# mit-acl/clipper

Hardware: AMD Instinct MI355X
Metric: affinity+solve ms and GEMV HBM GB/s, n=10k assoc, 95% outliers, 1/8 GPU (lower is better)
Workload: dtype f64 (M stored f32)

## Files before the change

### clipper_amd/csrc/k_affinity.hip.h

```cpp
#pragma once

#include <hip/hip_runtime.h>
#include <stdint.h>

#include "k_csc.hip.h"

namespace clipper_hip {


__global__ __launch_bounds__(256) void k_gather_points(const double* __restrict__ D, int d,
                                                        const int32_t* __restrict__ idx,
                                                        int64_t m, int64_t pstride,
                                                        double* __restrict__ P,
                                                        float* __restrict__ Pf) {
  const int64_t i = static_cast<int64_t>(blockIdx.x) * 256 + threadIdx.x;
  if (i >= pstride) return;
  const int64_t src = (i < m) ? idx[i] : 0;
  for (int k = 0; k < d; ++k) {
    const double v = (i < m) ? D[k + d * src] : 0.0;
    P[k * pstride + i] = v;
    Pf[k * pstride + i] = static_cast<float>(v);
  }
}

template <typename T>
__device__ __forceinline__ T store_score(double scr, double affinityeps) {
  if (!(scr > affinityeps)) return T(0);
  T v = static_cast<T>(scr);
  if (v == T(0)) v = static_cast<T>(1.17549435e-38);
  return v;
}

template <typename T>
__device__ __forceinline__ void store4(T* p, T a, T b, T c, T d);
template <>
__device__ __forceinline__ void store4<float>(float* p, float a, float b, float c, float d) {
  *reinterpret_cast<float4*>(p) = make_float4(a, b, c, d);
}
template <>
__device__ __forceinline__ void store4<double>(double* p, double a, double b, double c,
                                               double d) {
  *reinterpret_cast<double4*>(p) = make_double4(a, b, c, d);
}

struct EuclidParams {
  double sigma, epsilon, mindist, affinityeps;
};

template <typename T, int D>
__global__ __launch_bounds__(256) void k_affinity_euclid(
    T* __restrict__ S, int64_t ld, int64_t m, int64_t c0, int rows_per_blk, int d,
    const double* __restrict__ P1, const double* __restrict__ P2, int64_t pstride,
    const int32_t* __restrict__ A0, const int32_t* __restrict__ A1, EuclidParams prm) {
  const int64_t c = (static_cast<int64_t>(blockIdx.x) * 256 + threadIdx.x) * 4;
  if (c >= ld) return;
  const int64_t r0 = static_cast<int64_t>(blockIdx.y) * rows_per_blk;
  const int64_t r1 = (r0 + rows_per_blk < m) ? r0 + rows_per_blk : m;
  constexpr int DD = (D > 0) ? D : 1;

  int64_t gi[4];
  bool valid[4];
  int32_t a0c[4], a1c[4];
  double p1c[4][DD], p2c[4][DD];
#pragma unroll
  for (int q = 0; q < 4; ++q) {
    const int64_t g = c0 + c + q;
    valid[q] = g < m;
    gi[q] = valid[q] ? g : (m - 1);
    a0c[q] = A0[gi[q]];
    a1c[q] = A1[gi[q]];
    if (D > 0) {
#pragma unroll
      for (int k = 0; k < DD; ++k) {
        p1c[q][k] = P1[k * pstride + gi[q]];
        p2c[q][k] = P2[k * pstride + gi[q]];
      }
    }
  }

  for (int64_t r = r0; r < r1; ++r) {
    const int32_t a0r = A0[r], a1r = A1[r];
    double p1r[DD], p2r[DD];
    if (D > 0) {
#pragma unroll
      for (int k = 0; k < DD; ++k) {
        p1r[k] = P1[k * pstride + r];
        p2r[k] = P2[k * pstride + r];
      }
    }
    T out[4];
#pragma unroll
    for (int q = 0; q < 4; ++q) {
      double s1 = 0.0, s2 = 0.0;
      if (D > 0) {
#pragma unroll
        for (int k = 0; k < DD; ++k) {
          const double t1 = p1r[k] - p1c[q][k];
          const double t2 = p2r[k] - p2c[q][k];
          s1 = fma(t1, t1, s1);
          s2 = fma(t2, t2, s2);
        }
      } else {
        for (int k = 0; k < d; ++k) {
          const double t1 = P1[k * pstride + r] - P1[k * pstride + gi[q]];
          const double t2 = P2[k * pstride + r] - P2[k * pstride + gi[q]];
          s1 = fma(t1, t1, s1);
          s2 = fma(t2, t2, s2);
        }
      }
      const double l1 = sqrt(s1), l2 = sqrt(s2);
      bool ok = valid[q] && (a0r != a0c[q]) && (a1r != a1c[q]);
      if (prm.mindist > 0 && (l1 < prm.mindist || l2 < prm.mindist)) ok = false;
      const double cc = fabs(l1 - l2);
      double scr = 0.0;
      if (ok && cc < prm.epsilon) scr = exp(-0.5 * cc * cc / (prm.sigma * prm.sigma));
      out[q] = store_score<T>(scr, prm.affinityeps);
    }
    store4<T>(S + r * ld + c, out[0], out[1], out[2], out[3]);
  }
}

struct PointNormalParams {
  double sigp, epsp, sign, epsn, affinityeps;
};

template <typename T>
__global__ __launch_bounds__(256) void k_affinity_pointnormal(
    T* __restrict__ S, int64_t ld, int64_t m, int64_t c0, int rows_per_blk,
    const double* __restrict__ P1, const double* __restrict__ P2, int64_t pstride,
    const int32_t* __restrict__ A0, const int32_t* __restrict__ A1, PointNormalParams prm) {
  const int64_t c = (static_cast<int64_t>(blockIdx.x) * 256 + threadIdx.x) * 4;
  if (c >= ld) return;
  const int64_t r0 = static_cast<int64_t>(blockIdx.y) * rows_per_blk;
  const int64_t r1 = (r0 + rows_per_blk < m) ? r0 + rows_per_blk : m;

  bool valid[4];
  int32_t a0c[4], a1c[4];
  double p1c[4][6], p2c[4][6];
#pragma unroll
  for (int q = 0; q < 4; ++q) {
    const int64_t g = c0 + c + q;
    valid[q] = g < m;
    const int64_t gi = valid[q] ? g : (m - 1);
    a0c[q] = A0[gi];
    a1c[q] = A1[gi];
#pragma unroll
    for (int k = 0; k < 6; ++k) {
      p1c[q][k] = P1[k * pstride + gi];
      p2c[q][k] = P2[k * pstride + gi];
    }
  }

  for (int64_t r = r0; r < r1; ++r) {
    const int32_t a0r = A0[r], a1r = A1[r];
    double p1r[6], p2r[6];
#pragma unroll
    for (int k = 0; k < 6; ++k) {
      p1r[k] = P1[k * pstride + r];
      p2r[k] = P2[k * pstride + r];
    }
    T out[4];
#pragma unroll
    for (int q = 0; q < 4; ++q) {
      double s1 = 0.0, s2 = 0.0;
#pragma unroll
      for (int k = 0; k < 3; ++k) {
        const double t1 = p1r[k] - p1c[q][k];
        const double t2 = p2r[k] - p2c[q][k];
        s1 = fma(t1, t1, s1);
        s2 = fma(t2, t2, s2);
      }
      const double l1 = sqrt(s1), l2 = sqrt(s2);
      const double dot1 = fma(p1r[5], p1c[q][5], fma(p1r[4], p1c[q][4], p1r[3] * p1c[q][3]));
      const double dot2 = fma(p2r[5], p2c[q][5], fma(p2r[4], p2c[q][4], p2r[3] * p2c[q][3]));
      const bool ok = valid[q] && (a0r != a0c[q]) && (a1r != a1c[q]);
      double scr = 0.0;
      if (ok) {
        const double alpha1 = acos(dot1);
        const double alpha2 = acos(dot2);
        const double dp = fabs(l1 - l2);
        const double dn = fabs(alpha1 - alpha2);
        if (dp < prm.epsp && dn < prm.epsn) {
          const double sp = exp(-0.5 * dp * dp / (prm.sigp * prm.sigp));
          const double sn = exp(-0.5 * dn * dn / (prm.sign * prm.sign));
          scr = sp * sn;
        }
      }
      out[q] = store_score<T>(scr, prm.affinityeps);
    }
    store4<T>(S + r * ld + c, out[0], out[1], out[2], out[3]);
  }
}


constexpr int AFF_RG = 8;

__device__ __forceinline__ uint32_t lane_prefix(uint64_t mask) {
  return __builtin_amdgcn_mbcnt_hi(static_cast<uint32_t>(mask >> 32),
                                   __builtin_amdgcn_mbcnt_lo(static_cast<uint32_t>(mask), 0u));
}

__device__ __forceinline__ double pt_at(const double* __restrict__ P, uint32_t byte_off) {
  return *reinterpret_cast<const double*>(reinterpret_cast<const char*>(P) + byte_off);
}

template <typename T, int D>
__device__ __forceinline__ double exact_euclid_score(const double* __restrict__ P1,
                                                     const double* __restrict__ P2,
                                                     int64_t pstride, int64_t r, int64_t g,
                                                     const EuclidParams& prm) {
  const uint32_t pb = static_cast<uint32_t>(pstride) << 3, rb = static_cast<uint32_t>(r) << 3, gb = static_cast<uint32_t>(g) << 3;
  double s1 = 0.0, s2 = 0.0;
#pragma unroll
  for (int k = 0; k < D; ++k) {
    const double t1 = pt_at(P1, k * pb + rb) - pt_at(P1, k * pb + gb);
    const double t2 = pt_at(P2, k * pb + rb) - pt_at(P2, k * pb + gb);
    s1 = fma(t1, t1, s1);
    s2 = fma(t2, t2, s2);
  }
  const double l1 = sqrt(s1), l2 = sqrt(s2);
  if (prm.mindist > 0 && (l1 < prm.mindist || l2 < prm.mindist)) return 0.0;
  const double cc = fabs(l1 - l2);
  return (cc < prm.epsilon) ? exp(-0.5 * cc * cc / (prm.sigma * prm.sigma)) : 0.0;
}

template <typename T, int D>
__global__ __launch_bounds__(256) void k_affinity_euclid_compact(
    T* __restrict__ S, int64_t ld, int64_t m, int64_t c0, int rows_per_blk,
    const double* __restrict__ P1, const double* __restrict__ P2,
    const float* __restrict__ P1f, const float* __restrict__ P2f, int64_t pstride,
    const int32_t* __restrict__ A0, const int32_t* __restrict__ A1, EuclidParams prm,
    float eps_guarded) {
  __shared__ uint32_t queue[4][AFF_RG * 256];
  __shared__ T stage[4][AFF_RG][256];
  const int lane = threadIdx.x & 63;
  const int wave = __builtin_amdgcn_readfirstlane(threadIdx.x >> 6);
  const int64_t cw = static_cast<int64_t>(blockIdx.x) * 1024 + wave * 256;
  const int64_t c = cw + lane * 4;
  const int64_t r0 = static_cast<int64_t>(blockIdx.y) * rows_per_blk;
  const int64_t r1 = (r0 + rows_per_blk < m) ? r0 + rows_per_blk : m;
  if (cw >= ld) return;

  bool valid[4];
  int32_t a0c[4], a1c[4];
  float p1c[4][D], p2c[4][D];
#pragma unroll
  for (int q = 0; q < 4; ++q) {
    const int64_t g = c0 + c + q;
    valid[q] = (g < m) && (c + q < ld);
    const int64_t gi = (g < m) ? g : (m - 1);
    a0c[q] = A0[gi];
    a1c[q] = A1[gi];
#pragma unroll
    for (int k = 0; k < D; ++k) {
      p1c[q][k] = P1f[k * pstride + gi];
      p2c[q][k] = P2f[k * pstride + gi];
    }
  }
#pragma unroll
  for (int r8 = 0; r8 < AFF_RG; ++r8)
#pragma unroll
    for (int q = 0; q < 4; ++q) stage[wave][r8][lane * 4 + q] = T(0);

  for (int64_t base = r0; base < r1; base += AFF_RG) {
    uint32_t count = 0;
#pragma unroll
    for (int r8 = 0; r8 < AFF_RG; ++r8) {
      const int64_t r = base + r8;
      if (r < r1) {
        const int32_t a0r = A0[r], a1r = A1[r];
        float p1r[D], p2r[D];
#pragma unroll
        for (int k = 0; k < D; ++k) {
          p1r[k] = P1f[k * pstride + r];
          p2r[k] = P2f[k * pstride + r];
        }
#pragma unroll
        for (int q = 0; q < 4; ++q) {
          float s1 = 0.f, s2 = 0.f;
#pragma unroll
          for (int k = 0; k < D; ++k) {
            const float t1 = p1r[k] - p1c[q][k];
            const float t2 = p2r[k] - p2c[q][k];
            s1 = fmaf(t1, t1, s1);
            s2 = fmaf(t2, t2, s2);
          }
          const float cf = fabsf(__builtin_amdgcn_sqrtf(s1) - __builtin_amdgcn_sqrtf(s2));
          const bool cand = valid[q] && (a0r != a0c[q]) && (a1r != a1c[q]) && (cf < eps_guarded);
          const uint64_t mask = __ballot(cand);
          if (mask != 0) {
            if (cand) queue[wave][count + lane_prefix(mask)] =
                (static_cast<uint32_t>(r8) << 16) | static_cast<uint32_t>(lane * 4 + q);
            count += static_cast<uint32_t>(__popcll(mask));
          }
        }
      }
    }
    __builtin_amdgcn_fence(__ATOMIC_RELEASE, "wavefront");
    __builtin_amdgcn_wave_barrier();
    for (uint32_t e = lane; e < count; e += 64) {
      const uint32_t code = queue[wave][e];
      const int r8 = static_cast<int>(code >> 16);
      const int cl = static_cast<int>(code & 0xffffu);
      const double scr = exact_euclid_score<T, D>(P1, P2, pstride, base + r8, c0 + cw + cl, prm);
      stage[wave][r8][cl] = store_score<T>(scr, prm.affinityeps);
    }
    __builtin_amdgcn_fence(__ATOMIC_RELEASE, "wavefront");
    __builtin_amdgcn_wave_barrier();
    if (c < ld) {
#pragma unroll
      for (int r8 = 0; r8 < AFF_RG; ++r8) {
        const int64_t r = base + r8;
        if (r < r1) {
          T* sp = &stage[wave][r8][lane * 4];
          store4<T>(S + r * ld + c, sp[0], sp[1], sp[2], sp[3]);
          sp[0] = sp[1] = sp[2] = sp[3] = T(0);
        }
      }
    }
    __builtin_amdgcn_fence(__ATOMIC_RELEASE, "wavefront");
    __builtin_amdgcn_wave_barrier();
  }
}

template <typename T>
__device__ __forceinline__ double exact_pointnormal_score(const double* __restrict__ P1,
                                                          const double* __restrict__ P2,
                                                          int64_t pstride, int64_t r, int64_t g,
                                                          const PointNormalParams& prm) {
  const uint32_t pb = static_cast<uint32_t>(pstride) << 3, rb = static_cast<uint32_t>(r) << 3, gb = static_cast<uint32_t>(g) << 3;
  double p1r[6], p1g[6], p2r[6], p2g[6];
#pragma unroll
  for (int k = 0; k < 6; ++k) {
    p1r[k] = pt_at(P1, k * pb + rb);
    p1g[k] = pt_at(P1, k * pb + gb);
    p2r[k] = pt_at(P2, k * pb + rb);
    p2g[k] = pt_at(P2, k * pb + gb);
  }
  double s1 = 0.0, s2 = 0.0;
#pragma unroll
  for (int k = 0; k < 3; ++k) {
    const double t1 = p1r[k] - p1g[k];
    const double t2 = p2r[k] - p2g[k];
    s1 = fma(t1, t1, s1);
    s2 = fma(t2, t2, s2);
  }
  const double l1 = sqrt(s1), l2 = sqrt(s2);
  const double dot1 = fma(p1r[5], p1g[5], fma(p1r[4], p1g[4], p1r[3] * p1g[3]));
  const double dot2 = fma(p2r[5], p2g[5], fma(p2r[4], p2g[4], p2r[3] * p2g[3]));
  const double alpha1 = acos(dot1);
  const double alpha2 = acos(dot2);
  const double dp = fabs(l1 - l2);
  const double dn = fabs(alpha1 - alpha2);
  if (dp < prm.epsp && dn < prm.epsn) {
    const double sp = exp(-0.5 * dp * dp / (prm.sigp * prm.sigp));
    const double sn = exp(-0.5 * dn * dn / (prm.sign * prm.sign));
    return sp * sn;
  }
  return 0.0;
}

template <typename T>
__global__ __launch_bounds__(256) void k_affinity_pointnormal_compact(
    T* __restrict__ S, int64_t ld, int64_t m, int64_t c0, int rows_per_blk,
    const double* __restrict__ P1, const double* __restrict__ P2,
    const float* __restrict__ P1f, const float* __restrict__ P2f, int64_t pstride,
    const int32_t* __restrict__ A0, const int32_t* __restrict__ A1, PointNormalParams prm,
    float eps_guarded) {
  __shared__ uint32_t queue[4][AFF_RG * 256];
  __shared__ T stage[4][AFF_RG][256];
  const int lane = threadIdx.x & 63;
  const int wave = __builtin_amdgcn_readfirstlane(threadIdx.x >> 6);
  const int64_t cw = static_cast<int64_t>(blockIdx.x) * 1024 + wave * 256;
  const int64_t c = cw + lane * 4;
  const int64_t r0 = static_cast<int64_t>(blockIdx.y) * rows_per_blk;
  const int64_t r1 = (r0 + rows_per_blk < m) ? r0 + rows_per_blk : m;
  if (cw >= ld) return;

  bool valid[4];
  int32_t a0c[4], a1c[4];
  float p1c[4][3], p2c[4][3];
#pragma unroll
  for (int q = 0; q < 4; ++q) {
    const int64_t g = c0 + c + q;
    valid[q] = (g < m) && (c + q < ld);
    const int64_t gi = (g < m) ? g : (m - 1);
    a0c[q] = A0[gi];
    a1c[q] = A1[gi];
#pragma unroll
    for (int k = 0; k < 3; ++k) {
      p1c[q][k] = P1f[k * pstride + gi];
      p2c[q][k] = P2f[k * pstride + gi];
    }
  }
#pragma unroll
  for (int r8 = 0; r8 < AFF_RG; ++r8)
#pragma unroll
    for (int q = 0; q < 4; ++q) stage[wave][r8][lane * 4 + q] = T(0);

  for (int64_t base = r0; base < r1; base += AFF_RG) {
    uint32_t count = 0;
#pragma unroll
    for (int r8 = 0; r8 < AFF_RG; ++r8) {
      const int64_t r = base + r8;
      if (r < r1) {
        const int32_t a0r = A0[r], a1r = A1[r];
        float p1r[3], p2r[3];
#pragma unroll
        for (int k = 0; k < 3; ++k) {
          p1r[k] = P1f[k * pstride + r];
          p2r[k] = P2f[k * pstride + r];
        }
#pragma unroll
        for (int q = 0; q < 4; ++q) {
          float s1 = 0.f, s2 = 0.f;
#pragma unroll
          for (int k = 0; k < 3; ++k) {
            const float t1 = p1r[k] - p1c[q][k];
            const float t2 = p2r[k] - p2c[q][k];
            s1 = fmaf(t1, t1, s1);
            s2 = fmaf(t2, t2, s2);
          }
          const float dpf = fabsf(__builtin_amdgcn_sqrtf(s1) - __builtin_amdgcn_sqrtf(s2));
          const bool cand = valid[q] && (a0r != a0c[q]) && (a1r != a1c[q]) && (dpf < eps_guarded);
          const uint64_t mask = __ballot(cand);
          if (mask != 0) {
            if (cand) queue[wave][count + lane_prefix(mask)] =
                (static_cast<uint32_t>(r8) << 16) | static_cast<uint32_t>(lane * 4 + q);
            count += static_cast<uint32_t>(__popcll(mask));
          }
        }
      }
    }
    __builtin_amdgcn_fence(__ATOMIC_RELEASE, "wavefront");
    __builtin_amdgcn_wave_barrier();
    for (uint32_t e = lane; e < count; e += 64) {
      const uint32_t code = queue[wave][e];
      const int r8 = static_cast<int>(code >> 16);
      const int cl = static_cast<int>(code & 0xffffu);
      const double scr = exact_pointnormal_score<T>(P1, P2, pstride, base + r8, c0 + cw + cl, prm);
      stage[wave][r8][cl] = store_score<T>(scr, prm.affinityeps);
    }
    __builtin_amdgcn_fence(__ATOMIC_RELEASE, "wavefront");
    __builtin_amdgcn_wave_barrier();
    if (c < ld) {
#pragma unroll
      for (int r8 = 0; r8 < AFF_RG; ++r8) {
        const int64_t r = base + r8;
        if (r < r1) {
          T* sp = &stage[wave][r8][lane * 4];
          store4<T>(S + r * ld + c, sp[0], sp[1], sp[2], sp[3]);
          sp[0] = sp[1] = sp[2] = sp[3] = T(0);
        }
      }
    }
    __builtin_amdgcn_fence(__ATOMIC_RELEASE, "wavefront");
    __builtin_amdgcn_wave_barrier();
  }
}


constexpr int AT = 128;
constexpr int AT_PITCH = AT + 1;
#ifndef CLIPPER_AT_WAVES
#define CLIPPER_AT_WAVES 8
#endif
constexpr int AT_WAVES = CLIPPER_AT_WAVES;
constexpr int AT_ROWS_PER_WAVE = AT / AT_WAVES;
constexpr int AT_QUEUE = 256;
template <typename VT = float>
constexpr int at_sym_img_bytes() { return (AT * AT_PITCH * static_cast<int>(sizeof(VT)) + 15) / 16 * 16; }
constexpr int AT_SYM_MASK_BYTES = 2 * AT * 16;
template <typename VT = float>
constexpr int at_sym_lds_bytes() { return at_sym_img_bytes<VT>() + AT_WAVES * AT_QUEUE * 4 + AT_SYM_MASK_BYTES; }
constexpr int AT_SYM_IMG_BYTES = at_sym_img_bytes<float>();
constexpr int AT_SYM_LDS_BYTES = at_sym_lds_bytes<float>();

__device__ __forceinline__ void tile_of(int t, int nT, int& I, int& J) {
  const float b = 2.0f * nT + 1.0f;
  int i = static_cast<int>((b - sqrtf(b * b - 8.0f * static_cast<float>(t))) * 0.5f);
  if (i < 0) i = 0;
  if (i > nT - 1) i = nT - 1;
  while (i > 0 && i * nT - i * (i - 1) / 2 > t) --i;
  while (i + 1 < nT && (i + 1) * nT - (i + 1) * i / 2 <= t) ++i;
  I = i;
  J = i + (t - (i * nT - i * (i - 1) / 2));
}

template <int D, bool POINTNORMAL, typename VT = float>
__global__ __launch_bounds__(AT_WAVES * 64, AT_WAVES / 2) void k_affinity_sym(
    VT* __restrict__ S, int64_t ld, int64_t m, int nT, const double* __restrict__ P1,
    const double* __restrict__ P2, const float* __restrict__ P1f, const float* __restrict__ P2f,
    int64_t pstride, const int32_t* __restrict__ A0, const int32_t* __restrict__ A1,
    EuclidParams eprm, PointNormalParams nprm, float E2 ,
    CscOut O ) {
  extern __shared__ __attribute__((aligned(16))) char sym_smem[];
  const bool stamp = O.stamps != nullptr && blockIdx.x < 800 && threadIdx.x == 0;
  long long ts[5] = {0, 0, 0, 0, 0};
  if (stamp) ts[0] = wall_clock64();
  VT* img = reinterpret_cast<VT*>(sym_smem);
  constexpr int IMG_BYTES = at_sym_img_bytes<VT>();
  const int lane = threadIdx.x & 63;
  const int wave = __builtin_amdgcn_readfirstlane(threadIdx.x >> 6);
  uint32_t* queue = reinterpret_cast<uint32_t*>(sym_smem + IMG_BYTES) + wave * AT_QUEUE;
  int I, J;
  const int tb = static_cast<int>(blockIdx.x);
  tile_of((tb & 1) ? static_cast<int>(gridDim.x) - 1 - (tb >> 1) : (tb >> 1), nT, I, J);
  const int64_t r0 = static_cast<int64_t>(I) * AT, c0 = static_cast<int64_t>(J) * AT;
  const double affinityeps = POINTNORMAL ? nprm.affinityeps : eprm.affinityeps;

  bool validc[2];
  int32_t a0c[2], a1c[2];
  float p1c[2][D], p2c[2][D];
#pragma unroll
  for (int q = 0; q < 2; ++q) {
    const int64_t g = c0 + 2 * lane + q;
    validc[q] = g < m;
    const int64_t gi = validc[q] ? g : (m - 1);
    a0c[q] = A0[gi];
    a1c[q] = A1[gi];
#pragma unroll
    for (int k = 0; k < D; ++k) {
      p1c[q][k] = P1f[k * pstride + gi];
      p2c[q][k] = P2f[k * pstride + gi];
    }
  }
  uint32_t* colmask = reinterpret_cast<uint32_t*>(sym_smem + IMG_BYTES + AT_WAVES * AT_QUEUE * 4);
  uint32_t* rowmask = colmask + AT * 4;
  colmask[threadIdx.x] = 0;
  rowmask[threadIdx.x] = 0;
  if (S != nullptr) {
#pragma unroll 4
    for (int rr = 0; rr < AT_ROWS_PER_WAVE; ++rr) {
      VT* row = img + (wave * AT_ROWS_PER_WAVE + rr) * AT_PITCH;
      row[2 * lane] = VT(0);
      row[2 * lane + 1] = VT(0);
    }
  }
  __syncthreads();

  auto drain = [&](uint32_t head, uint32_t n) {
    if (lane < n) {
      const uint32_t code = queue[(head + lane) & (AT_QUEUE - 1)];
      const int rl = static_cast<int>(code >> 8);
      const int cl = static_cast<int>(code & 0xffu);
      double scr;
      if (POINTNORMAL) scr = exact_pointnormal_score<VT>(P1, P2, pstride, r0 + rl, c0 + cl, nprm);
      else scr = exact_euclid_score<VT, D>(P1, P2, pstride, r0 + rl, c0 + cl, eprm);
      const VT v = store_score<VT>(scr, affinityeps);
      img[rl * AT_PITCH + cl] = v;
      if (v != VT(0)) {
        atomicOr(&colmask[cl * 4 + (rl >> 5)], 1u << (rl & 31));
        atomicOr(&rowmask[rl * 4 + (cl >> 5)], 1u << (cl & 31));
      }
    }
  };

  uint32_t head = 0, tail = 0;
  int32_t va0, va1;
  float vp1[D], vp2[D];
  {
    const int64_t rw = r0 + wave * AT_ROWS_PER_WAVE + (lane < AT_ROWS_PER_WAVE ? lane : 0);
    const int64_t ri = rw < m ? rw : (m - 1);
    va0 = A0[ri];
    va1 = A1[ri];
#pragma unroll
    for (int k = 0; k < D; ++k) {
      vp1[k] = P1f[k * pstride + ri];
      vp2[k] = P2f[k * pstride + ri];
    }
  }
  for (int rr = 0; rr < AT_ROWS_PER_WAVE; ++rr) {
    const int rl = wave * AT_ROWS_PER_WAVE + rr;
    const int64_t r = r0 + rl;
    if (r < m) {
      const int32_t a0r = __builtin_amdgcn_readlane(va0, rr), a1r = __builtin_amdgcn_readlane(va1, rr);
      float p1r[D], p2r[D];
#pragma unroll
      for (int k = 0; k < D; ++k) {
        p1r[k] = __int_as_float(__builtin_amdgcn_readlane(__float_as_int(vp1[k]), rr));
        p2r[k] = __int_as_float(__builtin_amdgcn_readlane(__float_as_int(vp2[k]), rr));
      }
#pragma unroll
      for (int q = 0; q < 2; ++q) {
        float s1 = 0.f, s2 = 0.f;
#pragma unroll
        for (int k = 0; k < D; ++k) {
          const float t1 = p1r[k] - p1c[q][k];
          const float t2 = p2r[k] - p2c[q][k];
          s1 = fmaf(t1, t1, s1);
          s2 = fmaf(t2, t2, s2);
        }
        const float t = (s1 + s2) - E2;
        const bool close = (t <= 0.f) || (t * t < (4.0f * 1.0000038147f) * (s1 * s2));
        const bool cand = validc[q] && (a0r != a0c[q]) && (a1r != a1c[q]) && close;
        const uint64_t mask = __ballot(cand);
        if (mask != 0) {
          if (cand) queue[(tail + lane_prefix(mask)) & (AT_QUEUE - 1)] =
              (static_cast<uint32_t>(rl) << 8) | static_cast<uint32_t>(2 * lane + q);
          tail += static_cast<uint32_t>(__popcll(mask));
        }
      }
      if (tail - head >= 64) {
        __builtin_amdgcn_fence(__ATOMIC_RELEASE, "wavefront");
        __builtin_amdgcn_wave_barrier();
        while (tail - head >= 64) {
          drain(head, 64);
          head += 64;
        }
      }
    }
  }
  __builtin_amdgcn_fence(__ATOMIC_RELEASE, "wavefront");
  __builtin_amdgcn_wave_barrier();
  while (head < tail) {
    const uint32_t n = (tail - head < 64) ? tail - head : 64;
    drain(head, n);
    head += n;
  }
  if (stamp) ts[1] = wall_clock64();
  __syncthreads();

  if (O.Pre != nullptr) {
    static_assert(AT_WAVES == 8 && AT == SL_SUB && AT == 2 * SL_W, "four slices per tile");
    unsigned long long* base_s = reinterpret_cast<unsigned long long*>(sym_smem + IMG_BYTES);
    const int sl = wave & 3, half = wave >> 2;
    const int e = sl & 1;
    const bool mirror = sl >= 2;
    const VT* col = mirror ? img + (64 * e + lane) * AT_PITCH : img + 64 * e + lane;
    const uint4 mk = *reinterpret_cast<const uint4*>((mirror ? rowmask : colmask) + (64 * e + lane) * 4);
    const uint64_t mlo = static_cast<uint64_t>(mk.x) | (static_cast<uint64_t>(mk.y) << 32);
    const uint64_t mhi = static_cast<uint64_t>(mk.z) | (static_cast<uint64_t>(mk.w) << 32);
    const int cg = 2 * (mirror ? I : J) + e;
    const int k = mirror ? J : I;
    const int64_t s = (cg < O.ncg && k < O.nchunks && !(mirror && I == J))
                          ? static_cast<int64_t>(cg) * O.nchunks + k : -1;
    slice_emit_lds(col, mirror ? 1 : AT_PITCH, mlo, mhi, s, sl, half, O, base_s, stamp ? ts + 2 : nullptr);
    if (stamp) {
      ts[4] = wall_clock64();
      for (int i = 0; i < 5; ++i) O.stamps[blockIdx.x * 5 + i] = ts[i];
    }
  }

  if (S != nullptr && c0 + 2 * lane < ld) {
    for (int rr = 0; rr < AT_ROWS_PER_WAVE; ++rr) {
      const int rl = wave * AT_ROWS_PER_WAVE + rr;
      const int64_t r = r0 + rl;
      if (r < m) {
        const VT* row = img + rl * AT_PITCH + 2 * lane;
        if constexpr (sizeof(VT) == 4) *reinterpret_cast<float2*>(S + r * ld + c0 + 2 * lane) = make_float2(row[0], row[1]);
        else *reinterpret_cast<double2*>(S + r * ld + c0 + 2 * lane) = make_double2(row[0], row[1]);
      }
    }
  }
  if (S != nullptr && I != J && r0 + 2 * lane < ld) {
    for (int cc = 0; cc < AT_ROWS_PER_WAVE; ++cc) {
      const int cl = wave * AT_ROWS_PER_WAVE + cc;
      const int64_t c = c0 + cl;
      if (c < m) {
        const VT v0 = img[(2 * lane) * AT_PITCH + cl];
        const VT v1 = img[(2 * lane + 1) * AT_PITCH + cl];
        if constexpr (sizeof(VT) == 4) *reinterpret_cast<float2*>(S + c * ld + r0 + 2 * lane) = make_float2(v0, v1);
        else *reinterpret_cast<double2*>(S + c * ld + r0 + 2 * lane) = make_double2(v0, v1);
      }
    }
  }
}

struct RectGeom {
  int64_t m;
  int64_t nrows;
  const int32_t* rowmap;
  int64_t col0, ncols;
  int nTc;
  int64_t tile0;
};

template <typename VT>
constexpr int rect_tw() { return sizeof(VT) == 4 ? 128 : 64; }
template <typename VT, int TW = rect_tw<VT>()>
constexpr int rect_img_bytes() { return (AT * (TW + 1) * static_cast<int>(sizeof(VT)) + 15) / 16 * 16; }
template <typename VT, int TW = rect_tw<VT>()>
constexpr int rect_lds_bytes() {
  return rect_img_bytes<VT, TW>() + AT_WAVES * AT_QUEUE * 4 + TW * 16 + AT * 4;
}

template <int D, bool POINTNORMAL, typename VT, int TW = rect_tw<VT>()>
__global__ __launch_bounds__(AT_WAVES * 64, AT_WAVES / 2) void k_affinity_rect(
    RectGeom G, const double* __restrict__ P1, const double* __restrict__ P2,
    const float* __restrict__ P1f, const float* __restrict__ P2f, int64_t pstride,
    const int32_t* __restrict__ A0, const int32_t* __restrict__ A1, EuclidParams eprm,
    PointNormalParams nprm, float E2, SliceOut O) {
  constexpr int CPL = TW / 64;
  constexpr int PITCH = TW + 1;
  static_assert(AT_WAVES == 8 && AT == SL_SUB && (TW == 64 || TW == 128), "a tile is as tall as a slice");
  extern __shared__ __attribute__((aligned(16))) char rect_smem[];
  VT* img = reinterpret_cast<VT*>(rect_smem);
  const int lane = threadIdx.x & 63;
  const int wave = __builtin_amdgcn_readfirstlane(threadIdx.x >> 6);
  uint32_t* queue = reinterpret_cast<uint32_t*>(rect_smem + rect_img_bytes<VT, TW>()) + wave * AT_QUEUE;
  uint32_t* colmask = reinterpret_cast<uint32_t*>(rect_smem + rect_img_bytes<VT, TW>() + AT_WAVES * AT_QUEUE * 4);
  int32_t* rowidx = reinterpret_cast<int32_t*>(colmask + TW * 4);
  const int64_t tile = G.tile0 + blockIdx.x;
  const int I = static_cast<int>(tile / G.nTc);
  const int J = G.nTc - 1 - static_cast<int>(tile % G.nTc);
  const int64_t r0 = static_cast<int64_t>(I) * AT;
  const int64_t cl0 = static_cast<int64_t>(J) * TW;
  const double affinityeps = POINTNORMAL ? nprm.affinityeps : eprm.affinityeps;

  bool validc[CPL];
  int32_t a0c[CPL], a1c[CPL];
  float p1c[CPL][D], p2c[CPL][D];
#pragma unroll
  for (int q = 0; q < CPL; ++q) {
    const int64_t lc = cl0 + CPL * lane + q;
    const int64_t g = G.col0 + lc;
    validc[q] = lc < G.ncols && g < G.m;
    const int64_t gi = validc[q] ? g : (G.m - 1);
    a0c[q] = A0[gi];
    a1c[q] = A1[gi];
#pragma unroll
    for (int k = 0; k < D; ++k) {
      p1c[q][k] = P1f[k * pstride + gi];
      p2c[q][k] = P2f[k * pstride + gi];
    }
  }
  for (int t = threadIdx.x; t < TW * 4; t += AT_WAVES * 64) colmask[t] = 0;
  if (threadIdx.x < AT) {
    const int64_t r = r0 + threadIdx.x;
    const int64_t rc = r < G.nrows ? r : (G.nrows - 1);
    rowidx[threadIdx.x] = G.rowmap ? G.rowmap[rc] : static_cast<int32_t>(rc);
  }
  __syncthreads();

  auto drain = [&](uint32_t head, uint32_t n) {
    if (lane < n) {
      const uint32_t code = queue[(head + lane) & (AT_QUEUE - 1)];
      const int rl = static_cast<int>(code >> 8);
      const int cl = static_cast<int>(code & 0xffu);
      const int64_t ra = rowidx[rl], ca = G.col0 + cl0 + cl;
      double scr;
      if (POINTNORMAL) scr = exact_pointnormal_score<VT>(P1, P2, pstride, ra, ca, nprm);
      else scr = exact_euclid_score<VT, D>(P1, P2, pstride, ra, ca, eprm);
      const VT v = store_score<VT>(scr, affinityeps);
      if (v != VT(0)) {
        img[rl * PITCH + cl] = v;
        atomicOr(&colmask[cl * 4 + (rl >> 5)], 1u << (rl & 31));
      }
    }
  };

  uint32_t head = 0, tail = 0;
  int32_t va0, va1;
  float vp1[D], vp2[D];
  {
    const int ri = rowidx[wave * AT_ROWS_PER_WAVE + (lane < AT_ROWS_PER_WAVE ? lane : 0)];
    va0 = A0[ri];
    va1 = A1[ri];
#pragma unroll
    for (int k = 0; k < D; ++k) {
      vp1[k] = P1f[k * pstride + ri];
      vp2[k] = P2f[k * pstride + ri];
    }
  }
  for (int rr = 0; rr < AT_ROWS_PER_WAVE; ++rr) {
    const int rl = wave * AT_ROWS_PER_WAVE + rr;
    if (r0 + rl < G.nrows) {
      const int32_t a0r = __builtin_amdgcn_readlane(va0, rr), a1r = __builtin_amdgcn_readlane(va1, rr);
      float p1r[D], p2r[D];
#pragma unroll
      for (int k = 0; k < D; ++k) {
        p1r[k] = __int_as_float(__builtin_amdgcn_readlane(__float_as_int(vp1[k]), rr));
        p2r[k] = __int_as_float(__builtin_amdgcn_readlane(__float_as_int(vp2[k]), rr));
      }
#pragma unroll
      for (int q = 0; q < CPL; ++q) {
        float s1 = 0.f, s2 = 0.f;
#pragma unroll
        for (int k = 0; k < D; ++k) {
          const float t1 = p1r[k] - p1c[q][k];
          const float t2 = p2r[k] - p2c[q][k];
          s1 = fmaf(t1, t1, s1);
          s2 = fmaf(t2, t2, s2);
        }
        const float t = (s1 + s2) - E2;
        const bool close = (t <= 0.f) || (t * t < (4.0f * 1.0000038147f) * (s1 * s2));
        const bool cand = validc[q] && (a0r != a0c[q]) && (a1r != a1c[q]) && close;
        const uint64_t mask = __ballot(cand);
        if (mask != 0) {
          if (cand) queue[(tail + lane_prefix(mask)) & (AT_QUEUE - 1)] =
              (static_cast<uint32_t>(rl) << 8) | static_cast<uint32_t>(CPL * lane + q);
          tail += static_cast<uint32_t>(__popcll(mask));
        }
      }
      if (tail - head >= 64) {
        __builtin_amdgcn_fence(__ATOMIC_RELEASE, "wavefront");
        __builtin_amdgcn_wave_barrier();
        while (tail - head >= 64) {
          drain(head, 64);
          head += 64;
        }
      }
    }
  }
  __builtin_amdgcn_fence(__ATOMIC_RELEASE, "wavefront");
  __builtin_amdgcn_wave_barrier();
  while (head < tail) {
    const uint32_t n = (tail - head < 64) ? tail - head : 64;
    drain(head, n);
    head += n;
  }
  __syncthreads();

  unsigned long long* base_s = reinterpret_cast<unsigned long long*>(rect_smem + rect_img_bytes<VT, TW>());
  const int sl = wave & 3, half = wave >> 2;
  const int e = sl < CPL ? sl : 0;
  const VT* col = img + 64 * e + lane;
  const uint4 mk = *reinterpret_cast<const uint4*>(colmask + (64 * e + lane) * 4);
  const uint64_t mlo = static_cast<uint64_t>(mk.x) | (static_cast<uint64_t>(mk.y) << 32);
  const uint64_t mhi = static_cast<uint64_t>(mk.z) | (static_cast<uint64_t>(mk.w) << 32);
  const int cg = static_cast<int>(cl0 / 64) + e;
  const int64_t s = (sl < CPL && cg < O.ncg && I < O.nchunks) ? static_cast<int64_t>(cg) * O.nchunks + I : -1;
  slice_emit_lds<VT>(col, PITCH, mlo, mhi, s, sl, half, O, base_s, nullptr);
}

}
```

Measured before the change: 1.286.

## Stage tile row data in LDS records and shrink candidate queue to 16-bit

After: 1.272, median of 6. About the same (-1.1%).

```diff
diff --git a/clipper_amd/csrc/k_affinity.hip.h b/clipper_amd/csrc/k_affinity.hip.h
--- a/clipper_amd/csrc/k_affinity.hip.h
+++ b/clipper_amd/csrc/k_affinity.hip.h
@@ -468,11 +468,15 @@
 constexpr int AT_WAVES = CLIPPER_AT_WAVES;
 constexpr int AT_ROWS_PER_WAVE = AT / AT_WAVES;
 constexpr int AT_QUEUE = 256;
+constexpr int AT_QUEUE_BYTES = AT_WAVES * AT_QUEUE * 2;
+constexpr int AT_ROWREC_BYTES = AT * 32;
 template <typename VT = float>
 constexpr int at_sym_img_bytes() { return (AT * AT_PITCH * static_cast<int>(sizeof(VT)) + 15) / 16 * 16; }
 constexpr int AT_SYM_MASK_BYTES = 2 * AT * 16;
 template <typename VT = float>
-constexpr int at_sym_lds_bytes() { return at_sym_img_bytes<VT>() + AT_WAVES * AT_QUEUE * 4 + AT_SYM_MASK_BYTES; }
+constexpr int at_sym_lds_bytes() {
+  return at_sym_img_bytes<VT>() + AT_QUEUE_BYTES + AT_ROWREC_BYTES + AT_SYM_MASK_BYTES;
+}
 constexpr int AT_SYM_IMG_BYTES = at_sym_img_bytes<float>();
 constexpr int AT_SYM_LDS_BYTES = at_sym_lds_bytes<float>();
 
@@ -485,6 +489,91 @@
   while (i + 1 < nT && (i + 1) * nT - (i + 1) * i / 2 <= t) ++i;
   I = i;
   J = i + (t - (i * nT - i * (i - 1) / 2));
+}
+
+struct alignas(16) AtRowRec {
+  float p[6];
+  int32_t a0, a1;
+};
+static_assert(sizeof(AtRowRec) * AT == AT_ROWREC_BYTES, "two ds_read_b128 per row");
+
+template <int D>
+__device__ __forceinline__ void at_stage_row(AtRowRec* rec, int64_t i, const float* __restrict__ P1f,
+                                             const float* __restrict__ P2f, int64_t pstride,
+                                             const int32_t* __restrict__ A0,
+                                             const int32_t* __restrict__ A1) {
+  float p[6];
+#pragma unroll
+  for (int k = 0; k < 3; ++k) {
+    p[2 * k] = k < D ? P1f[k * pstride + i] : 0.f;
+    p[2 * k + 1] = k < D ? P2f[k * pstride + i] : 0.f;
+  }
+  float4* o = reinterpret_cast<float4*>(rec);
+  o[0] = make_float4(p[0], p[1], p[2], p[3]);
+  o[1] = make_float4(p[4], p[5], __int_as_float(A0[i]), __int_as_float(A1[i]));
+}
+
+template <int D, int CPL, typename Drain>
+__device__ __forceinline__ void at_score_rows(const AtRowRec* rec, int rl0, int nv,
+                                              const float (&p1c)[CPL][D], const float (&p2c)[CPL][D],
+                                              const int32_t (&a0c)[CPL], const int32_t (&a1c)[CPL],
+                                              const bool (&validc)[CPL], float E2, uint16_t* queue,
+                                              Drain&& drain) {
+  const int lane = threadIdx.x & 63;
+  uint32_t head = 0, tail = 0;
+  for (int rr = 0; rr < nv; ++rr) {
+    const int rl = rl0 + rr;
+    const float4 x = reinterpret_cast<const float4*>(rec + rl)[0];
+    const float4 y = reinterpret_cast<const float4*>(rec + rl)[1];
+    const float p1r[3] = {x.x, x.z, y.x}, p2r[3] = {x.y, x.w, y.y};
+    const int32_t a0r = __float_as_int(y.z), a1r = __float_as_int(y.w);
+    bool cand[CPL];
+    uint64_t mk[CPL], any = 0;
+#pragma unroll
+    for (int q = 0; q < CPL; ++q) {
+      float s1 = 0.f, s2 = 0.f;
+#pragma unroll
+      for (int k = 0; k < D; ++k) {
+        const float t1 = p1r[k] - p1c[q][k];
+        const float t2 = p2r[k] - p2c[q][k];
+        s1 = fmaf(t1, t1, s1);
+        s2 = fmaf(t2, t2, s2);
+      }
+      const float t = (s1 + s2) - E2;
+      const bool close = (t <= 0.f) | (t * t < (4.0f * 1.0000038147f) * (s1 * s2));
+      cand[q] = validc[q] & (a0r != a0c[q]) & (a1r != a1c[q]) & close;
+      mk[q] = __builtin_amdgcn_ballot_w64(cand[q]);
+      any |= mk[q];
+    }
+    if (any != 0) {
+      uint32_t slot = tail;
+#pragma unroll
+      for (int q = 0; q < CPL; ++q)
+        slot = __builtin_amdgcn_mbcnt_hi(static_cast<uint32_t>(mk[q] >> 32),
+                                         __builtin_amdgcn_mbcnt_lo(static_cast<uint32_t>(mk[q]), slot));
+#pragma unroll
+      for (int q = 0; q < CPL; ++q) {
+        if (cand[q]) queue[slot & (AT_QUEUE - 1)] = static_cast<uint16_t>((rl << 8) | (CPL * lane + q));
+        slot += cand[q] ? 1u : 0u;
+        tail += static_cast<uint32_t>(__popcll(mk[q]));
+      }
+      if (tail - head >= 64) {
+        __builtin_amdgcn_fence(__ATOMIC_RELEASE, "wavefront");
+        __builtin_amdgcn_wave_barrier();
+        while (tail - head >= 64) {
+          drain(head, 64u);
+          head += 64;
+        }
+      }
+    }
+  }
+  __builtin_amdgcn_fence(__ATOMIC_RELEASE, "wavefront");
+  __builtin_amdgcn_wave_barrier();
+  while (head < tail) {
+    const uint32_t n = (tail - head < 64) ? tail - head : 64;
+    drain(head, n);
+    head += n;
+  }
 }
 
 template <int D, bool POINTNORMAL, typename VT = float>
@@ -502,7 +591,8 @@
   constexpr int IMG_BYTES = at_sym_img_bytes<VT>();
   const int lane = threadIdx.x & 63;
   const int wave = __builtin_amdgcn_readfirstlane(threadIdx.x >> 6);
-  uint32_t* queue = reinterpret_cast<uint32_t*>(sym_smem + IMG_BYTES) + wave * AT_QUEUE;
+  uint16_t* queue = reinterpret_cast<uint16_t*>(sym_smem + IMG_BYTES) + wave * AT_QUEUE;
+  AtRowRec* rec = reinterpret_cast<AtRowRec*>(sym_smem + IMG_BYTES + AT_QUEUE_BYTES);
   int I, J;
   const int tb = static_cast<int>(blockIdx.x);
   tile_of((tb & 1) ? static_cast<int>(gridDim.x) - 1 - (tb >> 1) : (tb >> 1), nT, I, J);
@@ -525,10 +615,14 @@
       p2c[q][k] = P2f[k * pstride + gi];
     }
   }
-  uint32_t* colmask = reinterpret_cast<uint32_t*>(sym_smem + IMG_BYTES + AT_WAVES * AT_QUEUE * 4);
+  uint32_t* colmask = reinterpret_cast<uint32_t*>(sym_smem + IMG_BYTES + AT_QUEUE_BYTES + AT_ROWREC_BYTES);
   uint32_t* rowmask = colmask + AT * 4;
   colmask[threadIdx.x] = 0;
   rowmask[threadIdx.x] = 0;
+  if (threadIdx.x < AT) {
+    const int64_t r = r0 + threadIdx.x;
+    at_stage_row<D>(rec + threadIdx.x, r < m ? r : (m - 1), P1f, P2f, pstride, A0, A1);
+  }
   if (S != nullptr) {
 #pragma unroll 4
     for (int rr = 0; rr < AT_ROWS_PER_WAVE; ++rr) {
@@ -556,67 +650,10 @@
     }
   };
 
-  uint32_t head = 0, tail = 0;
-  int32_t va0, va1;
-  float vp1[D], vp2[D];
   {
-    const int64_t rw = r0 + wave * AT_ROWS_PER_WAVE + (lane < AT_ROWS_PER_WAVE ? lane : 0);
-    const int64_t ri = rw < m ? rw : (m - 1);
-    va0 = A0[ri];
-    va1 = A1[ri];
-#pragma unroll
-    for (int k = 0; k < D; ++k) {
-      vp1[k] = P1f[k * pstride + ri];
-      vp2[k] = P2f[k * pstride + ri];
-    }
-  }
-  for (int rr = 0; rr < AT_ROWS_PER_WAVE; ++rr) {
-    const int rl = wave * AT_ROWS_PER_WAVE + rr;
-    const int64_t r = r0 + rl;
-    if (r < m) {
-      const int32_t a0r = __builtin_amdgcn_readlane(va0, rr), a1r = __builtin_amdgcn_readlane(va1, rr);
-      float p1r[D], p2r[D];
-#pragma unroll
-      for (int k = 0; k < D; ++k) {
-        p1r[k] = __int_as_float(__builtin_amdgcn_readlane(__float_as_int(vp1[k]), rr));
-        p2r[k] = __int_as_float(__builtin_amdgcn_readlane(__float_as_int(vp2[k]), rr));
-      }
-#pragma unroll
-      for (int q = 0; q < 2; ++q) {
-        float s1 = 0.f, s2 = 0.f;
-#pragma unroll
-        for (int k = 0; k < D; ++k) {
-          const float t1 = p1r[k] - p1c[q][k];
-          const float t2 = p2r[k] - p2c[q][k];
-          s1 = fmaf(t1, t1, s1);
-          s2 = fmaf(t2, t2, s2);
-        }
-        const float t = (s1 + s2) - E2;
-        const bool close = (t <= 0.f) || (t * t < (4.0f * 1.0000038147f) * (s1 * s2));
-        const bool cand = validc[q] && (a0r != a0c[q]) && (a1r != a1c[q]) && close;
-        const uint64_t mask = __ballot(cand);
-        if (mask != 0) {
-          if (cand) queue[(tail + lane_prefix(mask)) & (AT_QUEUE - 1)] =
-              (static_cast<uint32_t>(rl) << 8) | static_cast<uint32_t>(2 * lane + q);
-          tail += static_cast<uint32_t>(__popcll(mask));
-        }
-      }
-      if (tail - head >= 64) {
-        __builtin_amdgcn_fence(__ATOMIC_RELEASE, "wavefront");
-        __builtin_amdgcn_wave_barrier();
-        while (tail - head >= 64) {
-          drain(head, 64);
-          head += 64;
-        }
-      }
-    }
-  }
-  __builtin_amdgcn_fence(__ATOMIC_RELEASE, "wavefront");
-  __builtin_amdgcn_wave_barrier();
-  while (head < tail) {
-    const uint32_t n = (tail - head < 64) ? tail - head : 64;
-    drain(head, n);
-    head += n;
+    const int64_t rw = r0 + wave * AT_ROWS_PER_WAVE;
+    const int nv = rw >= m ? 0 : (m - rw < AT_ROWS_PER_WAVE ? static_cast<int>(m - rw) : AT_ROWS_PER_WAVE);
+    at_score_rows<D, 2>(rec, wave * AT_ROWS_PER_WAVE, nv, p1c, p2c, a0c, a1c, validc, E2, queue, drain);
   }
   if (stamp) ts[1] = wall_clock64();
   __syncthreads();
@@ -682,7 +719,7 @@
 constexpr int rect_img_bytes() { return (AT * (TW + 1) * static_cast<int>(sizeof(VT)) + 15) / 16 * 16; }
 template <typename VT, int TW = rect_tw<VT>()>
 constexpr int rect_lds_bytes() {
-  return rect_img_bytes<VT, TW>() + AT_WAVES * AT_QUEUE * 4 + TW * 16 + AT * 4;
+  return rect_img_bytes<VT, TW>() + AT_QUEUE_BYTES + AT_ROWREC_BYTES + TW * 16 + AT * 4;
 }
 
 template <int D, bool POINTNORMAL, typename VT, int TW = rect_tw<VT>()>
@@ -698,8 +735,9 @@
   VT* img = reinterpret_cast<VT*>(rect_smem);
   const int lane = threadIdx.x & 63;
   const int wave = __builtin_amdgcn_readfirstlane(threadIdx.x >> 6);
-  uint32_t* queue = reinterpret_cast<uint32_t*>(rect_smem + rect_img_bytes<VT, TW>()) + wave * AT_QUEUE;
-  uint32_t* colmask = reinterpret_cast<uint32_t*>(rect_smem + rect_img_bytes<VT, TW>() + AT_WAVES * AT_QUEUE * 4);
+  uint16_t* queue = reinterpret_cast<uint16_t*>(rect_smem + rect_img_bytes<VT, TW>()) + wave * AT_QUEUE;
+  AtRowRec* rec = reinterpret_cast<AtRowRec*>(rect_smem + rect_img_bytes<VT, TW>() + AT_QUEUE_BYTES);
+  uint32_t* colmask = reinterpret_cast<uint32_t*>(rect_smem + rect_img_bytes<VT, TW>() + AT_QUEUE_BYTES + AT_ROWREC_BYTES);
   int32_t* rowidx = reinterpret_cast<int32_t*>(colmask + TW * 4);
   const int64_t tile = G.tile0 + blockIdx.x;
   const int I = static_cast<int>(tile / G.nTc);
@@ -729,7 +767,9 @@
   if (threadIdx.x < AT) {
     const int64_t r = r0 + threadIdx.x;
     const int64_t rc = r < G.nrows ? r : (G.nrows - 1);
-    rowidx[threadIdx.x] = G.rowmap ? G.rowmap[rc] : static_cast<int32_t>(rc);
+    const int32_t ri = G.rowmap ? G.rowmap[rc] : static_cast<int32_t>(rc);
+    rowidx[threadIdx.x] = ri;
+    at_stage_row<D>(rec + threadIdx.x, ri, P1f, P2f, pstride, A0, A1);
   }
   __syncthreads();
 
@@ -750,65 +790,10 @@
     }
   };
 
-  uint32_t head = 0, tail = 0;
-  int32_t va0, va1;
-  float vp1[D], vp2[D];
   {
-    const int ri = rowidx[wave * AT_ROWS_PER_WAVE + (lane < AT_ROWS_PER_WAVE ? lane : 0)];
-    va0 = A0[ri];
-    va1 = A1[ri];
-#pragma unroll
-    for (int k = 0; k < D; ++k) {
-      vp1[k] = P1f[k * pstride + ri];
-      vp2[k] = P2f[k * pstride + ri];
-    }
-  }
-  for (int rr = 0; rr < AT_ROWS_PER_WAVE; ++rr) {
-    const int rl = wave * AT_ROWS_PER_WAVE + rr;
-    if (r0 + rl < G.nrows) {
-      const int32_t a0r = __builtin_amdgcn_readlane(va0, rr), a1r = __builtin_amdgcn_readlane(va1, rr);
-      float p1r[D], p2r[D];
-#pragma unroll
-      for (int k = 0; k < D; ++k) {
-        p1r[k] = __int_as_float(__builtin_amdgcn_readlane(__float_as_int(vp1[k]), rr));
-        p2r[k] = __int_as_float(__builtin_amdgcn_readlane(__float_as_int(vp2[k]), rr));
-      }
-#pragma unroll
-      for (int q = 0; q < CPL; ++q) {
-        float s1 = 0.f, s2 = 0.f;
-#pragma unroll
-        for (int k = 0; k < D; ++k) {
-          const float t1 = p1r[k] - p1c[q][k];
-          const float t2 = p2r[k] - p2c[q][k];
-          s1 = fmaf(t1, t1, s1);
-          s2 = fmaf(t2, t2, s2);
-        }
-        const float t = (s1 + s2) - E2;
-        const bool close = (t <= 0.f) || (t * t < (4.0f * 1.0000038147f) * (s1 * s2));
-        const bool cand = validc[q] && (a0r != a0c[q]) && (a1r != a1c[q]) && close;
-        const uint64_t mask = __ballot(cand);
-        if (mask != 0) {
-          if (cand) queue[(tail + lane_prefix(mask)) & (AT_QUEUE - 1)] =
-              (static_cast<uint32_t>(rl) << 8) | static_cast<uint32_t>(CPL * lane + q);
-          tail += static_cast<uint32_t>(__popcll(mask));
-        }
-      }
-      if (tail - head >= 64) {
-        __builtin_amdgcn_fence(__ATOMIC_RELEASE, "wavefront");
-        __builtin_amdgcn_wave_barrier();
-        while (tail - head >= 64) {
-          drain(head, 64);
-          head += 64;
-        }
-      }
-    }
-  }
-  __builtin_amdgcn_fence(__ATOMIC_RELEASE, "wavefront");
-  __builtin_amdgcn_wave_barrier();
-  while (head < tail) {
-    const uint32_t n = (tail - head < 64) ? tail - head : 64;
-    drain(head, n);
-    head += n;
+    const int64_t rw = r0 + wave * AT_ROWS_PER_WAVE;
+    const int nv = rw >= G.nrows ? 0 : (G.nrows - rw < AT_ROWS_PER_WAVE ? static_cast<int>(G.nrows - rw) : AT_ROWS_PER_WAVE);
+    at_score_rows<D, CPL>(rec, wave * AT_ROWS_PER_WAVE, nv, p1c, p2c, a0c, a1c, validc, E2, queue, drain);
   }
   __syncthreads();
 
```
